# Vi-Sri/CerebralSignalNetworks

Hardware: AMD Instinct MI355X
Metric: EEG-segments/sec training (128ch x 500, hidden=768) (higher is better)
Workload: dtype bf16

## Files before the change

### cerebralsignalnetworks_amd/csrc/csn_common.h

```cpp
#pragma once
#include <hip/hip_runtime.h>
#include <stdint.h>
#include <stdio.h>
#include <stdlib.h>
#include <atomic>
#include <string>

#include "../../include/csn_hip.h"

namespace csn {

typedef __bf16 bf16_t;
typedef __attribute__((ext_vector_type(8))) __bf16 bf16x8;
typedef __attribute__((ext_vector_type(4))) __bf16 bf16x4;
typedef __attribute__((ext_vector_type(4))) float f32x4;
typedef __attribute__((ext_vector_type(4))) short s16x4;

void set_error(const std::string& msg);
int fail(int status, const char* fmt, ...);

#define CSN_HIP_CHECK(expr)                                                              \
  do {                                                                                   \
    hipError_t _e = (expr);                                                              \
    if (_e != hipSuccess)                                                                \
      return ::csn::fail(CSN_ERR_HIP, "%s failed: %s (%s:%d)", #expr, hipGetErrorString(_e), \
                         __FILE__, __LINE__);                                            \
  } while (0)

#define CSN_LAUNCH_CHECK()                                                               \
  do {                                                                                   \
    hipError_t _e = hipGetLastError();                                                   \
    if (_e != hipSuccess)                                                                \
      return ::csn::fail(CSN_ERR_HIP, "kernel launch failed: %s (%s:%d)",                \
                         hipGetErrorString(_e), __FILE__, __LINE__);                     \
  } while (0)

#define CSN_REQUIRE(cond, ...)                                                           \
  do {                                                                                   \
    if (!(cond)) return ::csn::fail(CSN_ERR_INVALID_ARGUMENT, __VA_ARGS__);              \
  } while (0)

struct Options {
  bool cell_v1, no_persist, no_persist_bwd, persist_streams, no_xcd_local, no_rotate, no_fuse_x, no_beside,
      no_side_stream, fwd_ksplit, fwd_nsplit, fwd_flags, bwd_flags, dpoll_no_hint, fwd_hint, gemm_no_dma, gemm_no_256, gemm_generic, tn_no_tr, tn_no_stagger, filter_v1, tags_no_rearm, gemm_no_192, no_half_tiles, nt_no_w4, no_fwd_park;
  int chunk;
  int tn_stages;
};
static inline Options options_from_env() {
  auto on = [](const char* name) { return getenv(name) != nullptr; };
  auto num = [](const char* name, int dflt) {
    const char* e = getenv(name);
    return e ? atoi(e) : dflt;
  };
  Options o{};
  o.cell_v1 = on("CSN_CELL_V1");
  o.no_persist = on("CSN_NO_PERSIST");
  o.no_persist_bwd = on("CSN_NO_PERSIST_BWD");
  o.persist_streams = on("CSN_PERSIST_STREAMS");
  o.no_xcd_local = on("CSN_NO_XCD_LOCAL");
  o.no_rotate = on("CSN_NO_ROTATE");
  o.no_fuse_x = on("CSN_NO_FUSE_X");
  o.no_beside = on("CSN_NO_BESIDE");
  o.no_half_tiles = on("CSN_NO_HALF_TILES");
  o.no_fwd_park = on("CSN_NO_FWD_PARK");
  o.no_side_stream = on("CSN_NO_SIDE_STREAM");
  o.fwd_ksplit = on("CSN_FWD_KSPLIT");
  o.fwd_nsplit = on("CSN_FWD_NSPLIT");
  o.fwd_flags = on("CSN_FWD_FLAGS");
  o.bwd_flags = on("CSN_BWD_FLAGS");
  o.dpoll_no_hint = on("CSN_DPOLL_NO_HINT");
  o.fwd_hint = on("CSN_FWD_HINT");
  o.tn_no_stagger = on("CSN_TN_NO_STAGGER");
  o.gemm_no_dma = on("CSN_GEMM_NO_DMA");
  o.gemm_no_256 = on("CSN_GEMM_NO_256");
  o.gemm_no_192 = on("CSN_GEMM_NO_192");
  o.nt_no_w4 = on("CSN_NT_NO_W4");
  o.gemm_generic = on("CSN_GEMM_GENERIC");
  o.tn_no_tr = on("CSN_TN_NO_TR");
  o.filter_v1 = on("CSN_FILTER_V1");
#ifdef CSN_SLAB_TAGS
  o.tags_no_rearm = on("CSN_TAGS_NO_REARM");
#endif
  o.chunk = num("CSN_LSTM_CHUNK", 32);
  if (o.chunk < 1) o.chunk = 1;
  o.tn_stages = num("CSN_TN_STAGES", 4);
  return o;
}
// ... 73 lines not shown
```

### cerebralsignalnetworks_amd/csrc/lstm.hip

```cpp
#include <algorithm>
#include <cstring>
#include <vector>

#include "csn_common.h"
#include "lstm_cell_blk.h"
#include "lstm_cell_common.h"
#include "lstm_dropout.h"
#include "lstm_f32_persist.h"
#include "lstm_resident.h"

namespace csn {

struct LayerWs {
  size_t wih, whh, whht, wiht, whh_blk, whht_blk, bias, xproj, gates, c_all, h_all, dgates, dx, dc_carry, hblk[2],
      dgblk[2], h_blk_all, counters, dg_blk_all, bflags;
  size_t h_drop;
};
struct WsLayout {
  LayerWs layer[8];
  size_t x_c, x_blk, wih0_blk, dy_tm, tn_scratch, colsum, status, agree, agree_b, zeros_bh, f32_bias_part, total;
  size_t zero_fwd, zero_fwd_bytes, zero_bwd, zero_bwd_bytes;
  bool fuse_x;
  bool il, persist, persist_bwd;
  bool fwd_ns;
  bool f32_persist;
};

static bool whole_chip() {
  int dev = 0, cus = 0;
  if (hipGetDevice(&dev) != hipSuccess) return false;
  return hipDeviceGetAttribute(&cus, hipDeviceAttributeMultiprocessorCount, dev) == hipSuccess && cus >= 256;
}

static WsLayout make_layout(const csnLstmDesc& d, int training, bool dropout, const Options& opt) {
  WsLayout w{};
  w.il = cell_blk_supported(d.H, d.dtype, opt);
  const bool slabs_fit = ((size_t)d.T + 1) * (((size_t)d.B + 63) / 64 * 64) * (size_t)d.H * 8 < ((size_t)1 << 32);
  w.fwd_ns = w.il && fwd_ns_supported(d.B, d.H, d.dtype, opt) && d.L <= 4;
  w.persist = w.fwd_ns || (w.il && slabs_fit && fwd_persist_supported(d.B, d.H, d.dtype, opt) && d.L <= 4);
  w.persist_bwd = w.persist && slabs_fit && training && bwd_persist_supported(d.B, d.H, d.dtype, opt);
  size_t off = 0;
  const size_t es = dtype_size(d.dtype);
  auto take = [&](size_t bytes) {
    size_t o = off;
    off += align_up(bytes, 256);
    return o;
  };
  const size_t TB = (size_t)d.T * d.B, H = d.H, G = 4 * (size_t)d.H;
  const size_t Bpad = ((size_t)d.B + 63) / 64 * 64;
  size_t tn_bytes = 0;
  for (int l = 0; l < d.L; ++l) {
    const size_t I = l == 0 ? d.I : d.H;
    LayerWs& L = w.layer[l];
    L.wih = take(G * I * es);
    L.wiht = take(G * I * es);
    L.bias = take(G * 4);
    if (w.il) {
      L.whh_blk = take(G * H * 2);
      L.whht_blk = take(G * H * 2);
      L.hblk[0] = take(Bpad * H * 2);
      L.hblk[1] = take(Bpad * H * 2);
      if (w.persist) L.h_blk_all = take(((size_t)(d.T < 3 ? 3 : d.T) + 1) * Bpad * H * 2);
    } else {
      L.whh = take(G * H * es);
      L.whht = take(G * H * es);
    }
    L.xproj = take(TB * G * 4);
    L.gates = take(TB * G * es);
    L.c_all = take((TB + d.B) * H * 4);
    L.h_all = take((TB + d.B) * H * es);
    if (training) {
      L.dgates = take(TB * G * es);
      L.dx = take(TB * I * 4);
      if (!w.persist_bwd) L.dc_carry = take((size_t)d.B * H * 4);
      if (w.il) {
        L.dgblk[0] = take(Bpad * G * 2);
        L.dgblk[1] = take(Bpad * G * 2);
      }
      if (w.persist_bwd) L.dg_blk_all = take((size_t)(d.T < 4 ? 4 : d.T) * Bpad * G * 2);
    }
    size_t a = gemm_tn_scratch_bytes(G, I, TB, opt), b = gemm_tn_scratch_bytes(G, H, TB, opt);
    if (a > tn_bytes) tn_bytes = a;
    if (b > tn_bytes) tn_bytes = b;
  }
  w.x_c = take(TB * d.I * es);
  w.status = take(256);
  w.fuse_x = w.persist && !opt.no_fuse_x &&
             (w.fwd_ns ? d.I == 128 : (d.I % 32 == 0 && d.I <= 128 && d.H != 512));
  if (w.fuse_x) {
    w.x_blk = take((size_t)d.T * Bpad * d.I * 2);
    w.wih0_blk = take(G * d.I * 2);
  }
  if (w.persist_bwd) w.zeros_bh = take((size_t)d.B * H * 4);
  w.f32_persist = !w.il && d.dtype == CSN_F32 && !opt.no_persist && !opt.cell_v1 && f32_persist_supported(d.B, d.H) && whole_chip();
  if (w.f32_persist) {
    const size_t MTt = Bpad / 64;
    w.zero_fwd = off;
    for (int l = 0; l < d.L; ++l) w.layer[l].counters = take(((size_t)d.T + 1) * MTt * kF32FlagLine * 4);
    w.zero_fwd_bytes = off - w.zero_fwd;
    for (int l = 0; l < d.L; ++l) w.layer[l].h_blk_all = take(((size_t)d.T + 1) * Bpad * H * 4);
    if (training) {
      for (int l = 0; l < d.L; ++l) w.layer[l].dg_blk_all = take((size_t)d.T * Bpad * G * 4);
      w.zeros_bh = take((size_t)d.B * H * 4);
      w.f32_bias_part = take(MTt * 4 * G * 4);
      w.zero_bwd = off;
// ... 2 lines not shown
    }
  }
  if (w.persist) {
    w.zero_fwd = off;
    for (int l = 0; l < d.L; ++l) w.layer[l].counters = take(((size_t)d.T + 1) * (Bpad / 64) * 4 * kPersistFlagLine * 4);
    w.agree = take(((size_t)d.T + 8) * 8 * sizeof(unsigned long long));
    w.zero_fwd_bytes = off - w.zero_fwd;
  }
  if (w.persist_bwd) {
    w.zero_bwd = off;
    for (int l = 0; l < d.L; ++l) {
      w.layer[l].dc_carry = take((size_t)d.B * H * 4);
      w.layer[l].bflags = take((size_t)d.T * (Bpad / 64) * 3 * kPersistFlagLine * 4);
    }
    w.agree_b = take(((size_t)d.T + 8) * 8 * sizeof(unsigned long long));
    w.zero_bwd_bytes = off - w.zero_bwd;
  }
  if (training) {
    w.dy_tm = take(TB * H * 4);
    w.tn_scratch = take(tn_bytes);
    w.colsum = take(colsum_scratch_bytes(G));
  }
  for (int l = 0; dropout && l + 1 < d.L; ++l) w.layer[l].h_drop = take(TB * H * es);
  w.total = off;
  return w;
}

static const int kPlanBits = CSN_LSTM_STATE | CSN_LSTM_DROPOUT | CSN_LSTM_REVERSE | CSN_LSTM_RESIDENT;

static int check_resident(const char* fn, const csnLstmDesc* d, int training) {
  if ((training & CSN_LSTM_RESIDENT) && !resident_supported(d->H))
    return fail(CSN_ERR_UNSUPPORTED, "%s: CSN_LSTM_RESIDENT takes H <= %d, not H=%d", fn, kResidentMaxH, d->H);
  return CSN_OK;
}
static void resident_options(Options& opt) {
  opt.cell_v1 = true;
  opt.no_persist = true;
}

static int check_desc(const char* fn, const csnLstmDesc* d) {
  CSN_REQUIRE(d != nullptr, "%s: null descriptor", fn);
  CSN_REQUIRE(d->B > 0 && d->T > 0 && d->I > 0 && d->H > 0, "%s: bad shape B=%d T=%d I=%d H=%d", fn, d->B, d->T,
              d->I, d->H);
  CSN_REQUIRE(d->L >= 1 && d->L <= 8, "%s: L=%d outside 1..8", fn, d->L);
  CSN_REQUIRE(d->H % 32 == 0, "%s: H=%d must be a multiple of 32", fn, d->H);
  CSN_REQUIRE(d->dtype == CSN_F32 || d->dtype == CSN_BF16, "%s: bad dtype %d", fn, d->dtype);
// ... 681 lines not shown
  return CSN_OK;
}

static bool drop_on(const Call& C) { return C.P.dropout && C.P.drop_p > 0.f && C.NL > 1; }
static const void* layer_input(const Call& C, int l) {
  if (l > 0 && drop_on(C)) return C.ws + C.w.layer[l - 1].h_drop;
  return l == 0 ? (const void*)(C.ws + C.w.x_c) : (const void*)(C.ws + C.w.layer[l - 1].h_all + (size_t)C.B * C.H * C.es);
}

static int drop_fwd(const Call& C, int l, int t_lo, int t_hi, hipStream_t on) {
  if (!drop_on(C)) return CSN_OK;
  const size_t BH = (size_t)C.B * C.H;
  return launch_lstm_dropout_fwd(C.ws + C.w.layer[l].h_all + (size_t)(t_lo + 1) * BH * C.es, C.ws + C.w.layer[l].h_drop + (size_t)t_lo * BH * C.es,
                                 (int64_t)(t_hi - t_lo + 1) * (int64_t)BH, ((uint64_t)l * C.T_full + t_lo) * BH, C.dt,
                                 dropout_cfg(C.P.drop_p, C.P.drop_seed, C.P.drop_subsequence), on);
}
static int drop_bwd(const Call& C, int l, int t_lo, int t_hi, hipStream_t on) {
  if (!drop_on(C)) return CSN_OK;
  const size_t BH = (size_t)C.B * C.H;
  return launch_lstm_dropout_bwd((float*)(C.ws + C.w.layer[l + 1].dx) + (size_t)t_lo * BH, (int64_t)(t_hi - t_lo + 1) * (int64_t)BH,
                                 ((uint64_t)l * C.T_full + t_lo) * BH, dropout_cfg(C.P.drop_p, C.P.drop_seed, C.P.drop_subsequence), on);
}

static int install_slot0(const Call& C, int l, const float* h0, const float* c0) {
  const LayerWs& L = C.w.layer[l];
  const size_t BH = (size_t)C.B * C.H;
  if (h0) {
    if (int rc = launch_cast(h0 + l * BH, C.ws + L.h_all, (int64_t)BH, C.dt, C.st)) return rc;
  } else {
    CSN_HIP_CHECK(hipMemsetAsync(C.ws + L.h_all, 0, BH * C.es, C.st));
  }
  if (c0)
    CSN_HIP_CHECK(hipMemcpyAsync(C.ws + L.c_all, c0 + l * BH, BH * 4, hipMemcpyDeviceToDevice, C.st));
  else
    CSN_HIP_CHECK(hipMemsetAsync(C.ws + L.c_all, 0, BH * 4, C.st));
  return CSN_OK;
}

static int seed_dc_carry(const Call& C, int l, const float* dc_n, bool zeroed) {
  const size_t BH = (size_t)C.B * C.H;
  if (dc_n)
    CSN_HIP_CHECK(hipMemcpyAsync(C.ws + C.w.layer[l].dc_carry, dc_n + l * BH, BH * 4, hipMemcpyDeviceToDevice, C.st));
  else if (!zeroed)
    CSN_HIP_CHECK(hipMemsetAsync(C.ws + C.w.layer[l].dc_carry, 0, BH * 4, C.st));
  return CSN_OK;
}

static int prep_row_major(const Call& C, const FwdArgs& A) {
  const WsLayout& w = C.w;
  char* ws = C.ws;
  hipStream_t st = C.st;
  const int H = C.H, dt = C.dt;
  const int64_t G = C.G;
  int rc;
  if ((rc = launch_cast_strided(A.x, A.xsb, A.xst, C.B, C.T, C.d.I, ws + w.x_c, dt, st, C.dlen, C.P.reverse, C.vrow, C.vt0))) return rc;
  if ((rc = mask_x(C, st))) return rc;
  for (int l = 0; l < C.NL; ++l) {
// ... 46 lines not shown

static int weight_grads_rm(const Call& C, const BwdArgs& A, int l, bool colsum) {
  const WsLayout& w = C.w;
  const LayerWs& L = w.layer[l];
  char* ws = C.ws;
  const int acc = C.P.grad_accumulate;
  int rc;
  if ((rc = gemm_tn_full(ws + L.dgates, ws + L.h_all, A.dw_hh[l], C.G, C.H, C.TB, C.dt, ws + w.tn_scratch, acc, C.st, C.P.opt))) return rc;
  if ((rc = gemm_tn_full(ws + L.dgates, layer_input(C, l), A.dw_ih[l], C.G, C.in_width(l), C.TB, C.dt, ws + w.tn_scratch, acc, C.st, C.P.opt))) return rc;
  if (colsum) return launch_colsum(ws + L.dgates, C.TB, C.G, C.dt, A.db_ih[l], A.db_hh[l], acc, ws + w.colsum, C.st);
  return CSN_OK;
}

static int weight_grads_blk(const Call& C, const BwdArgs& A, int l, hipStream_t on) {
  const WsLayout& w = C.w;
  const LayerWs& L = w.layer[l];
  char* ws = C.ws;
  const int H = C.H;
  const int64_t G = C.G, TB = C.TB, I = C.in_width(l);
  float* slabs = (float*)(ws + w.tn_scratch);
  const int acc = C.P.grad_accumulate;
  int S = 1, r;
  int cs_done = 0, S_cs = 1;
  if ((r = launch_gemm_tn_slabs(ws + L.dgates, ws + L.h_all, slabs, G, H, TB, CSN_BF16, on, &S, (float*)(ws + w.colsum), &cs_done, C.P.opt))) return r;
  S_cs = S;
  if ((r = launch_reduce_slabs_unperm(slabs, G * H, S, H, H, A.dw_hh[l], nullptr, acc, on))) return r;
  if ((r = launch_gemm_tn_slabs(ws + L.dgates, layer_input(C, l), slabs, G, I, TB, CSN_BF16, on, &S, nullptr, nullptr, C.P.opt))) return r;
  if ((r = launch_reduce_slabs_unperm(slabs, G * I, S, H, I, A.dw_ih[l], nullptr, acc, on))) return r;
  if (!cs_done) {
    if ((r = launch_colsum_partial(ws + L.dgates, TB, G, CSN_BF16, ws + w.colsum, on))) return r;
    S_cs = colsum_chunks();
  }
  return launch_reduce_slabs_unperm((const float*)(ws + w.colsum), G, S_cs, H, 1, A.db_ih[l], A.db_hh[l], acc, on);
}

static int prof_end(Call& C, int k, int launches, int cells) {
  Prof& g_prof = C.P.prof;
  if (int rc = prof_mark(g_prof, 2 * k + 1, C.st)) return rc;
  g_prof.launches[k] = launches;
  g_prof.cells[k] = cells;
  g_prof.have[k] = g_prof.on;
  return CSN_OK;
}

static int launch_dh0(const Call& C, int l, float* out) {
  const LayerWs& L = C.w.layer[l];
// ... 262 lines not shown
    a.B = B; a.T = T; a.MT_total = MTt;
    for (int m = 0; m < MTt; m += per) {
      a.mt0 = m;
      a.MT = MTt - m < per ? MTt - m : per;
      if ((rc = prof_pair(g_prof, 1, false, st))) return rc;
      if ((rc = launch_bwd_f32_persist(a, H, st))) return rc;
      if ((rc = prof_pair(g_prof, 1, true, st))) return rc;
      ++n_launch;
    }
    sum_rows_kernel<<<(unsigned)((G + 255) / 256), 256, 0, st>>>((const float*)(ws + w.f32_bias_part), MTt * 4, G, A.db_ih[l], A.db_hh[l], C.P.grad_accumulate);
    CSN_LAUNCH_CHECK();
    if (l > 0 && (rc = gemm_nt(ws + L.dgates, ws + L.wiht, nullptr, ws + L.dx, C.TB, H, G, CSN_F32, CSN_F32, 0, st, C.P.opt))) return rc;
    if (l > 0 && (rc = drop_bwd(C, l - 1, 0, T - 1, st))) return rc;
  }
  if ((rc = prof_end(C, 1, n_launch, T * NL))) return rc;
  for (int l = NL - 1; l >= 0; --l) {
    if ((rc = weight_grads_rm(C, A, l, false))) return rc;
    C.P.grads_ready(l);
  }
  if (A.dx) return dx_out(C, A.dx, st);
  return CSN_OK;
}

static int prep_fast(Call& C, const FwdArgs& A) {
  const csnLstmDesc& d = C.d;
  const WsLayout& w = C.w;
  char* ws = C.ws;
  hipStream_t st = C.st;
  const int B = C.B, T = C.T, H = C.H, NL = C.NL;
  const int64_t G = C.G, TB = C.TB;
  const size_t Bpad = ((size_t)B + 63) / 64 * 64;
  int rc;
  PrepArgs pa{};
  pa.vrow = C.vrow;
  pa.vt0 = C.vt0;
  int prep_rc = CSN_OK;
  auto job = [&](int kind, const float* a_, const float* b_, void* dst, int64_t n0, int64_t n1, int64_t n2, int64_t s0,
                 int64_t s1, int64_t Hh, int pr, int pk, int64_t work) {
    if (prep_rc != CSN_OK) return;
    if (pa.njobs == kPrepMaxJobs) {
      if ((prep_rc = launch_prep_multi(pa, st)) != CSN_OK) return;
      pa.njobs = 0;
    }
    PrepJob& J = pa.job[pa.njobs++];
    J = PrepJob{kind, a_, b_, dst, n0, n1, n2, s0, s1, Hh, pr, pk, work, 0u, 0u, nullptr};
  };
  job(kPrepCastX, A.x, nullptr, ws + w.x_c, B, T, d.I, A.xsb, A.xst, 0, C.P.reverse, 0, TB * d.I);
  pa.job[pa.njobs - 1].len = C.dlen;
  for (int l = 0; l < NL; ++l) {
    const LayerWs& L = w.layer[l];
    const int64_t I = C.in_width(l);
    job(kPrepPermRows, A.w_ih[l], nullptr, ws + L.wih, 0, I, 0, 0, 0, H, 0, 0, G * I);
    job(kPrepBlockify, A.w_hh[l], nullptr, ws + L.whh_blk, G, H, 0, H, 1, H, 1, 0, G * H / 8);
    job(kPrepBias, A.b_ih[l], A.b_hh[l], ws + L.bias, 0, 0, 0, 0, 0, H, 0, 0, G);
    if (C.P.training) {
      job(kPrepTransPerm, A.w_ih[l], nullptr, ws + L.wiht, 0, I, 0, 0, 0, H, 0, 0, G * I);
      job(kPrepBlockify, A.w_hh[l], nullptr, ws + L.whht_blk, H, G, 0, 1, H, H, 0, 1, H * G / 8);
    }
    if (!w.persist) {
      CSN_HIP_CHECK(hipMemsetAsync(ws + L.hblk[0], 0, Bpad * H * 2, st));
      CSN_HIP_CHECK(hipMemsetAsync(ws + L.hblk[1], 0, Bpad * H * 2, st));
      if (A.h0 && (rc = launch_blockify_x(A.h0 + (size_t)l * B * H, H, 0, B, 1, H, ws + L.hblk[0], st))) return rc;
      if ((rc = install_slot0(C, l, A.h0, A.c0))) return rc;
    }
  }
  if (w.fuse_x) {
    job(kPrepBlockifyX, A.x, nullptr, ws + w.x_blk, B, T, d.I, A.xsb, A.xst, (int64_t)Bpad, C.P.reverse, 0, (int64_t)T * Bpad * d.I / 8);
    pa.job[pa.njobs - 1].len = C.dlen;
    job(kPrepBlockify, A.w_ih[0], nullptr, ws + w.wih0_blk, G, d.I, 0, d.I, 1, H, 1, 0, G * d.I / 8);
  }
  if (prep_rc != CSN_OK) return prep_rc;
  if ((rc = launch_prep_multi(pa, st))) return rc;
  if ((rc = mask_x(C, st))) return rc;
  if (!w.fuse_x) {
    if ((rc = gemm_nt(ws + w.x_c, ws + w.layer[0].wih, (const float*)(ws + w.layer[0].bias), ws + w.layer[0].xproj,
                      TB, G, d.I, CSN_BF16, CSN_F32, 0, st, C.P.opt)))
      return rc;
  }
  return CSN_OK;
}

static int forward_il(Call& C, const FwdArgs& A) {
  const WsLayout& w = C.w;
  char* ws = C.ws;
  hipStream_t st = C.st;
  SideCtx* sc = &C.P.sc;
  int rc;
  if ((rc = side_ctx(C.P.sc))) return rc;
  hipStream_t side = C.P.opt.no_side_stream ? st : sc->side;
  const int B = C.B, T = C.T, H = C.H, NL = C.NL;
  const int64_t G = C.G;
  const int Cz = C.Cz, lag = 2 * Cz;
  const int training = C.P.training;
// ... 47 lines not shown
      xproj_ready[(size_t)(l + 1) * nch + c] = ev;
    }
  }
  return prof_end(C, 0, n_launch, n_cells);
}

static int forward_persist(Call& C, const FwdArgs& A) {
  Plan& P = C.P;
  const WsLayout& w = C.w;
  Prof& g_prof = P.prof;
  char* ws = C.ws;
  hipStream_t st = C.st;
  SideCtx* sc = &P.sc;
  int rc;
  if ((rc = side_ctx(P.sc))) return rc;
  hipStream_t side = P.opt.no_side_stream ? st : sc->side;
  const float* h0 = A.h0;
  const float* c0 = A.c0;
  const int B = C.B, T = C.T, H = C.H, NL = C.NL;
  const int Bpad = (B + 63) / 64 * 64, MT = Bpad / 64;
  const int Cz = C.Cz;
  const int nch = (T + Cz - 1) / Cz;
  const int training = P.training;
  if ((rc = prep_fast(C, A))) return rc;
  CSN_HIP_CHECK(hipMemsetAsync(ws + w.zero_fwd, 0, w.zero_fwd_bytes, st));
  auto fill_slot = [&](PersistFwdSlot& S, int l, int c) {
    const LayerWs& L = w.layer[l];
    S.w_blk = (const bf16_t*)(ws + L.whh_blk);
    S.xproj = (const float*)(ws + L.xproj);
    S.gates = training ? (bf16_t*)(ws + L.gates) : nullptr;
    S.c_all = (float*)(ws + L.c_all);
    S.h_all = (bf16_t*)(ws + L.h_all);
    S.h_blk_all = (bf16_t*)(ws + L.h_blk_all);
    S.flags = (unsigned*)(ws + L.counters);
    S.x_blk = nullptr;
    S.wih_blk = nullptr;
    S.bias = nullptr;
    S.I = 0;
    if (l == 0 && w.fuse_x) {
      S.x_blk = (const bf16_t*)(ws + w.x_blk);
      S.wih_blk = (const bf16_t*)(ws + w.wih0_blk);
      S.bias = (const float*)(ws + L.bias);
      S.I = C.d.I;
    }
    const Chunk k = chunk_at(C, c);
    S.t0 = k.t0;
    S.nsteps = k.nsteps;
  };
  PersistFwdArgs a{};
  a.error_flag = (unsigned*)(ws + w.status);
  a.B = B; a.H = H; a.T = T; a.Bpad = Bpad; a.MT = MT;
  a.rotate = !P.opt.no_rotate;
  a.park = !P.opt.no_fwd_park;
  a.data_polls = (!w.fwd_ns && !P.opt.fwd_flags) ? (P.opt.fwd_hint && !P.opt.dpoll_no_hint ? 1 : 2) : 0;
#ifdef CSN_SLAB_TAGS
  if (a.data_polls && P.opt.tags_no_rearm) a.data_polls |= 4;
#endif
  if (a.data_polls)
    for (int l = 0; l < NL; ++l)
      CSN_HIP_CHECK(hipMemsetAsync(ws + w.layer[l].h_blk_all, 0xff, (size_t)4 * Bpad * H * 2, st));
  a.state = (h0 || c0) ? 1 : 0;
  if (a.state) P.state_seen = true;
  for (int l = 0; l < NL && P.state_seen; ++l) {
    const LayerWs& L = w.layer[l];
    if (h0) {
      if ((rc = launch_blockify_x(h0 + (size_t)l * B * H, H, 0, B, 1, H, ws + L.h_blk_all, st))) return rc;
    } else if (a.state) {
      CSN_HIP_CHECK(hipMemsetAsync(ws + L.h_blk_all, 0, (size_t)Bpad * H * 2, st));
    }
    if ((rc = install_slot0(C, l, h0, c0))) return rc;
  }
  int n_launch = 0;
  P.half_launches[0] = 0;

  const int max_slots = NL < nch ? NL : nch;
  const int fwd_slices = w.fwd_ns ? fwd_ns_slices(H) : fwd_persist_slices(H);
  auto launch_fwd = [&](const PersistFwdArgs& args, hipStream_t on) {
    return w.fwd_ns ? launch_fwd_ns(args, on) : launch_fwd_persist(args, on);
  };
  const bool grouped = max_slots <= 4 && max_slots * MT <= 8 && fwd_slices <= 32 &&
                       !P.opt.persist_streams;
  if (grouped) {
    const int ndiag = nch + NL - 1;
    const bool try_local = !P.opt.no_xcd_local;
    if ((rc = prof_mark(g_prof, 0, st))) return rc;
    for (int dg = 0; dg < ndiag; ++dg) {
      int lay[4], chk[4], ns = 0;
      for (int l = 0; l < NL; ++l) {
        const int c = dg - l;
        if (c < 0 || c >= nch) continue;
        lay[ns] = l;
        chk[ns] = c;
        fill_slot(a.slot[ns], l, c);
// ... 141 lines not shown
  }
  if ((rc = prof_end(C, 1, n_launch, n_cells))) return rc;
  if ((rc = hand_off(sc, side, st))) return rc;
  for (int l = NL - 1; l >= 0; --l) C.P.grads_ready(l);
  return CSN_OK;
}

static int backward_persist(Call& C, const BwdArgs& A) {
  Plan& P = C.P;
  const WsLayout& w = C.w;
  Prof& g_prof = P.prof;
  char* ws = C.ws;
  hipStream_t st = C.st;
  const float* dh_n = A.dh_n;
  const int B = C.B, T = C.T, H = C.H, NL = C.NL;
  const int64_t G = C.G;
  const int Bpad = (B + 63) / 64 * 64, MT = Bpad / 64;
  const int Cz = C.Cz;
  const int nch = (T + Cz - 1) / Cz;
  const bool beside = NL > 1 && NL <= 4 && bwd_persist_slices(H) <= 28 && G % 64 == 0 && !P.opt.no_beside;
  const int lag = beside ? 2 : 1;
  const int ndiag = nch + lag * (NL - 1);
  int rc;
  CSN_HIP_CHECK(hipMemsetAsync(ws + w.zero_bwd, 0, w.zero_bwd_bytes, st));
  for (int l = 0; l < NL; ++l)
    if ((rc = seed_dc_carry(C, l, A.dc_n, true))) return rc;
  struct DhAdd { int l, t_lo, t_hi; };
  auto add_dh_n = [&](const DhAdd& q) -> int {
    return add_dh_n_rows(C, dh_n + (size_t)(q.l - 1) * B * H, (float*)(ws + w.layer[q.l].dx), q.t_lo, q.t_hi, st);
  };
  const bool try_local = !P.opt.no_xcd_local;

  PersistBwdArgs a{};
  a.error_flag = (unsigned*)(ws + w.status);
  a.B = B; a.H = H; a.T = T; a.Bpad = Bpad; a.MT = MT;
  a.xcd_groups = 1;
  a.grid_slices = 32;
  a.rotate = !P.opt.no_rotate;
  a.data_polls = P.opt.bwd_flags ? 0 : (P.opt.dpoll_no_hint ? 2 : 1);
#ifdef CSN_SLAB_TAGS
  if (a.data_polls && P.opt.tags_no_rearm) a.data_polls |= 4;
#endif
  P.dgates_copies = 2;
  if (a.data_polls)
    for (int l = 0; l < NL; ++l) CSN_HIP_CHECK(hipMemsetAsync(ws + w.layer[l].dg_blk_all, 0xff, (size_t)4 * Bpad * G * 2, st));
  int n_launch = 0;
  P.half_launches[1] = 0;
  BesideGemm pending[3];
  DhAdd pending_add[3] = {{0, 0, 0}, {0, 0, 0}, {0, 0, 0}};
  DhAdd pending_drop[3] = {{0, 0, 0}, {0, 0, 0}, {0, 0, 0}};
  int npending = 0;
  if ((rc = prof_mark(g_prof, 2, st))) return rc;
  for (int dg = 0; dg < ndiag; ++dg) {
    int lay[4], chk[4], ns = 0;
    for (int l = NL - 1; l >= 0; --l) {
      const int c = dg - lag * (NL - 1 - l);
      if (c < 0 || c >= nch) continue;
      const LayerWs& L = w.layer[l];
      PersistBwdSlot& S = a.slot[ns];
      S.wt_blk = (const bf16_t*)(ws + L.whht_blk);
      S.gates = (const bf16_t*)(ws + L.gates);
      S.c_all = (const float*)(ws + L.c_all);
      if (l == NL - 1) {
        S.dy = A.dy_tm;
        S.dy_last = A.dy_tm ? nullptr : A.dy_last;
      } else {
        S.dy = (const float*)(ws + w.layer[l + 1].dx);
// ... 330 lines not shown
```

### cerebralsignalnetworks_amd/csrc/lstm_cell_blk.h

```cpp
#pragma once
#include "csn_common.h"

#ifdef CSN_SLAB_TAGS
#define CSN_DPOLL_MODE(x) ((x) & 3)
#define CSN_DPOLL_NO_REARM(x) (((x) & 4) != 0)
#else
#define CSN_DPOLL_MODE(x) (x)
#define CSN_DPOLL_NO_REARM(x) false
#endif

namespace csn {

struct CellFwdProb {
  const bf16_t* h_prev_blk;
  const bf16_t* w_blk;
  const float* xproj;
  const float* c_prev;
  bf16_t* gates_out;
  float* c_out;
  bf16_t* h_out;
  bf16_t* h_out_blk;
};
struct CellFwdArgs {
  CellFwdProb p[4];
// ... 74 lines not shown
  bf16_t* dgates;
  bf16_t* dg_blk_all;
  unsigned* flags;
  int t_hi, nsteps;
};
struct PersistBwdArgs {
  PersistBwdSlot slot[4];
  int nslots;
  BesideGemm gemm[3];
  int ngemm;
  int grid_slices;
  int xcd_groups;
  int rotate;
  int data_polls;
  unsigned long long* agree;
  unsigned* error_flag;
  int B, H, T, Bpad, MT;
  int half_tiles;
};
bool bwd_persist_supported(int B, int H, int dtype, const Options& opt);
int bwd_persist_slices(int H);
int launch_bwd_persist(const PersistBwdArgs& a, hipStream_t st, const int* lengths = nullptr);

enum { kPrepBlockify = 0, kPrepPermRows, kPrepTransPerm, kPrepBias, kPrepCastX, kPrepBlockifyX };
static constexpr int kPrepMaxJobs = 32;
struct PrepJob {
  int kind;
  const float* a;
  const float* b;
  void* dst;
  int64_t n0, n1, n2, s0, s1, H;
  int perm_r, perm_k;
  int64_t work;
  unsigned blk_begin, blk_count;
  const int* len;
};
struct PrepArgs {
  PrepJob job[kPrepMaxJobs];
  int njobs;
  const int* vrow;
  const int* vt0;
};
static_assert(sizeof(PrepArgs) <= 4096, "PrepArgs is passed by value: the kernel-argument segment holds 4096 bytes");
int launch_prep_multi(PrepArgs& A, hipStream_t st);

bool cell_blk_supported(int H, int dtype, const Options& opt);
int launch_cell_fwd_il(const CellFwdArgs& a, int nprob, hipStream_t st);
int launch_cell_bwd_il(const CellBwdArgs& a, int nprob, hipStream_t st, const CellMask* mask = nullptr);
int launch_blockify_x(const float* x, int64_t xsb, int64_t xst, int B, int T, int I, void* dst, hipStream_t st);
int launch_blockify(const float* src, int64_t ld_r, int64_t ld_k, int64_t R, int64_t K, int perm_r, int perm_k,
                    int64_t H, void* dst, hipStream_t st);
int launch_permute_rows_cast(const float* src, int64_t H, int64_t I, void* dst, hipStream_t st);
int launch_transpose_perm_cast(const float* src, int64_t H, int64_t I, void* dst, hipStream_t st);
int launch_bias_perm_sum(const float* a, const float* b, int64_t H, float* dst, hipStream_t st);
int launch_reduce_slabs_unperm(const float* slabs, int64_t slab_stride, int S, int64_t H, int64_t C, float* out,
                               float* out2, int accumulate, hipStream_t st);

}
```

### cerebralsignalnetworks_amd/csrc/lstm_cell_blk.hip

```cpp
#include "csn_common.h"
#include "lstm_cell_common.h"
#include "lstm_cell_blk.h"

#ifdef CSN_STAMPS
__device__ unsigned long long* g_stamps = nullptr;
#define CSN_STAMP(i)                                                                      \
  do {                                                                                    \
    __builtin_amdgcn_sched_barrier(0);                                                    \
    if (threadIdx.x == 0)                                                                 \
      g_stamps[((blockIdx.z * gridDim.y + blockIdx.y) * gridDim.x + blockIdx.x) * 8 + (i)] = wall_clock64(); \
    __builtin_amdgcn_sched_barrier(0);                                                    \
  } while (0)
#else
#define CSN_STAMP(i)
#endif

namespace csn {

__device__ __forceinline__ int64_t std_row(int64_t nprime, int64_t H) { return (nprime & 3) * H + (nprime >> 2); }

__global__ void __launch_bounds__(256)
blockify_cast_kernel(const float* __restrict__ src, int64_t ld_r, int64_t ld_k, int64_t R, int64_t K, int perm_r,
                     int perm_k, int64_t H, bf16_t* __restrict__ dst) {
  const int64_t nchunks = R * K / 8;
// ... 30 lines not shown
    const int64_t c = i / G, n = i % G;
    dst[i] = (bf16_t)src[std_row(n, H) * I + c];
  }
}

__global__ void bias_perm_sum_kernel(const float* __restrict__ a, const float* __restrict__ b, int64_t H,
                                     float* __restrict__ dst) {
  const int64_t i = (int64_t)blockIdx.x * blockDim.x + threadIdx.x;
  if (i < 4 * H) dst[i] = a[std_row(i, H)] + b[std_row(i, H)];
}

__global__ void reduce_slabs_unperm_kernel(const float* __restrict__ slabs, int64_t slab_stride, int S, int64_t H,
                                           int64_t C, float* out, float* out2, int accumulate) {
  const int64_t total = 4 * H * C;
  const int64_t stride = (int64_t)gridDim.x * blockDim.x;
  for (int64_t i = (int64_t)blockIdx.x * blockDim.x + threadIdx.x; i < total; i += stride) {
    const int64_t n = i / C, c = i % C;
    float acc = 0.0f;
    for (int s = 0; s < S; ++s) acc += slabs[(int64_t)s * slab_stride + i];
    const int64_t o = std_row(n, H) * C + c;
    out[o] = accumulate ? out[o] + acc : acc;
    if (out2 != nullptr) out2[o] = accumulate ? out2[o] + acc : acc;
  }
}

__global__ void __launch_bounds__(256) prep_multi_kernel(PrepArgs A) {
  __shared__ __attribute__((aligned(16))) bf16_t tp[64][72];
  int j = 0;
  while (j + 1 < A.njobs && blockIdx.x >= A.job[j + 1].blk_begin) ++j;
  const PrepJob& J = A.job[j];
  const int64_t vb = blockIdx.x - J.blk_begin, vg = J.blk_count;
  const int64_t gid = vb * blockDim.x + threadIdx.x, stride = vg * blockDim.x;
  switch (J.kind) {
    case kPrepBlockify: {
      const int64_t R = J.n0, K = J.n1, H = J.H, ld_r = J.s0, ld_k = J.s1, kblocks = K >> 5;
      bf16_t* dst = (bf16_t*)J.dst;
      if (J.perm_k && !J.perm_r && ld_r == 1 && (R & 63) == 0 && (K & 63) == 0 && (ld_k & 3) == 0) {
        const int64_t tiles_u = R >> 6, ntiles = tiles_u * (K >> 6);
        const int t = threadIdx.x, rr = t >> 2, seg = t & 3;
        for (int64_t tile = vb; tile < ntiles; tile += vg) {
          const int64_t tu = tile % tiles_u, tk = tile / tiles_u;
          const float4* sp = reinterpret_cast<const float4*>(J.a + std_row(tk * 64 + rr, H) * ld_k + tu * 64 + seg * 16);
          const float4 q0 = sp[0], q1 = sp[1], q2 = sp[2], q3 = sp[3];
          *reinterpret_cast<bf16x8*>(&tp[rr][seg * 16]) = (bf16x8){(bf16_t)q0.x, (bf16_t)q0.y, (bf16_t)q0.z, (bf16_t)q0.w, (bf16_t)q1.x, (bf16_t)q1.y, (bf16_t)q1.z, (bf16_t)q1.w};
          *reinterpret_cast<bf16x8*>(&tp[rr][seg * 16 + 8]) = (bf16x8){(bf16_t)q2.x, (bf16_t)q2.y, (bf16_t)q2.z, (bf16_t)q2.w, (bf16_t)q3.x, (bf16_t)q3.y, (bf16_t)q3.z, (bf16_t)q3.w};
          __syncthreads();
// ... 130 lines not shown
          if (J.perm_r) t = n - 1 - t;
          if (t < 0 || (win && t >= n)) {
            *reinterpret_cast<uint4*>(dst + ci * 8) = make_uint4(0u, 0u, 0u, 0u);
            continue;
          }
          if (win) {
            sr = A.vrow[r];
            t += A.vt0[r];
          }
        }
        bf16x8 v;
        if (r < Bn && ((J.s0 | J.s1) & 3) == 0 && (reinterpret_cast<uintptr_t>(J.a) & 15) == 0) {
          const float4* sp = reinterpret_cast<const float4*>(J.a + sr * J.s0 + t * J.s1 + k);
          const float4 u = sp[0], w = sp[1];
          v = (bf16x8){(bf16_t)u.x, (bf16_t)u.y, (bf16_t)u.z, (bf16_t)u.w, (bf16_t)w.x, (bf16_t)w.y, (bf16_t)w.z, (bf16_t)w.w};
        } else {
#pragma unroll
          for (int e = 0; e < 8; ++e) v[e] = (bf16_t)(r < Bn ? J.a[sr * J.s0 + t * J.s1 + k + e] : 0.f);
        }
        *reinterpret_cast<bf16x8*>(dst + ci * 8) = v;
      }
      break;
    }
  }
}

int launch_prep_multi(PrepArgs& A, hipStream_t st) {
  CSN_REQUIRE(A.njobs >= 1 && A.njobs <= kPrepMaxJobs, "launch_prep_multi: %d jobs", A.njobs);
  unsigned total = 0;
  for (int j = 0; j < A.njobs; ++j) {
    int64_t blocks = (A.job[j].work + 255) / 256;
    if (blocks < 1) blocks = 1;
    if (blocks > 2048) blocks = 2048;
    A.job[j].blk_begin = total;
    A.job[j].blk_count = (unsigned)blocks;
    total += (unsigned)blocks;
  }
  prep_multi_kernel<<<total, 256, 0, st>>>(A);
  CSN_LAUNCH_CHECK();
  return CSN_OK;
}

static inline unsigned cap_grid(int64_t n) {
  int64_t g = (n + 255) / 256;
  return (unsigned)(g < 1 ? 1 : (g > 2048 ? 2048 : g));
}

// ... 381 lines not shown
```

Before: 27960.

## Fuse workspace memsets into prep kernel and batch weight-gradient slab reductions

Folds the forward workspace zero/0xff memsets into the existing multi-job prep kernel, and merges the backward memsets into a single multi-region fill kernel. In the backward weight-gradient path, both TN GEMMs now write to separate slab buffers so that the dW_hh, dW_ih and bias reductions run in one launch with a vectorized slab-sum kernel. This aims to cut the launch count and serialization per step, at the cost of an extra scratch buffer and more complex job dispatch.

New measurement: 27900 (median of 2 runs). About the same (-0.2%).

```diff
diff --git a/cerebralsignalnetworks_amd/csrc/csn_common.h b/cerebralsignalnetworks_amd/csrc/csn_common.h
--- a/cerebralsignalnetworks_amd/csrc/csn_common.h
+++ b/cerebralsignalnetworks_amd/csrc/csn_common.h
@@ -42,7 +42,7 @@
 
 struct Options {
   bool cell_v1, no_persist, no_persist_bwd, persist_streams, no_xcd_local, no_rotate, no_fuse_x, no_beside,
-      no_side_stream, fwd_ksplit, fwd_nsplit, fwd_flags, bwd_flags, dpoll_no_hint, fwd_hint, gemm_no_dma, gemm_no_256, gemm_generic, tn_no_tr, tn_no_stagger, filter_v1, tags_no_rearm, gemm_no_192, no_half_tiles, nt_no_w4, no_fwd_park;
+      no_side_stream, fwd_ksplit, fwd_nsplit, fwd_flags, bwd_flags, dpoll_no_hint, fwd_hint, gemm_no_dma, gemm_no_256, gemm_generic, tn_no_tr, tn_no_stagger, filter_v1, tags_no_rearm, gemm_no_192, no_half_tiles, nt_no_w4, no_fwd_park, no_fill_fuse, no_reduce_fuse;
   int chunk;
   int tn_stages;
 };
@@ -63,6 +63,8 @@
   o.no_beside = on("CSN_NO_BESIDE");
   o.no_half_tiles = on("CSN_NO_HALF_TILES");
   o.no_fwd_park = on("CSN_NO_FWD_PARK");
+  o.no_fill_fuse = on("CSN_NO_FILL_FUSE");
+  o.no_reduce_fuse = on("CSN_NO_REDUCE_FUSE");
   o.no_side_stream = on("CSN_NO_SIDE_STREAM");
   o.fwd_ksplit = on("CSN_FWD_KSPLIT");
   o.fwd_nsplit = on("CSN_FWD_NSPLIT");
diff --git a/cerebralsignalnetworks_amd/csrc/lstm.hip b/cerebralsignalnetworks_amd/csrc/lstm.hip
--- a/cerebralsignalnetworks_amd/csrc/lstm.hip
+++ b/cerebralsignalnetworks_amd/csrc/lstm.hip
@@ -19,6 +19,7 @@
 struct WsLayout {
   LayerWs layer[8];
   size_t x_c, x_blk, wih0_blk, dy_tm, tn_scratch, colsum, status, agree, agree_b, zeros_bh, f32_bias_part, total;
+  size_t tn_scratch2;
   size_t zero_fwd, zero_fwd_bytes, zero_bwd, zero_bwd_bytes;
   bool fuse_x;
   bool il, persist, persist_bwd;
@@ -48,7 +49,7 @@
   };
   const size_t TB = (size_t)d.T * d.B, H = d.H, G = 4 * (size_t)d.H;
   const size_t Bpad = ((size_t)d.B + 63) / 64 * 64;
-  size_t tn_bytes = 0;
+  size_t tn_bytes = 0, tn2_bytes = 0;
   for (int l = 0; l < d.L; ++l) {
     const size_t I = l == 0 ? d.I : d.H;
     LayerWs& L = w.layer[l];
@@ -81,6 +82,7 @@
     }
     size_t a = gemm_tn_scratch_bytes(G, I, TB, opt), b = gemm_tn_scratch_bytes(G, H, TB, opt);
     if (a > tn_bytes) tn_bytes = a;
+    if (a > tn2_bytes) tn2_bytes = a;
     if (b > tn_bytes) tn_bytes = b;
   }
   w.x_c = take(TB * d.I * es);
@@ -129,6 +131,7 @@
     w.colsum = take(colsum_scratch_bytes(G));
   }
   for (int l = 0; dropout && l + 1 < d.L; ++l) w.layer[l].h_drop = take(TB * H * es);
+  if (w.persist_bwd && !opt.no_reduce_fuse) w.tn_scratch2 = take(tn2_bytes);
   w.total = off;
   return w;
 }
@@ -856,17 +859,17 @@
                                  ((uint64_t)l * C.T_full + t_lo) * BH, dropout_cfg(C.P.drop_p, C.P.drop_seed, C.P.drop_subsequence), on);
 }
 
-static int install_slot0(const Call& C, int l, const float* h0, const float* c0) {
+static int install_slot0(const Call& C, int l, const float* h0, const float* c0, bool zeroed = false) {
   const LayerWs& L = C.w.layer[l];
   const size_t BH = (size_t)C.B * C.H;
   if (h0) {
     if (int rc = launch_cast(h0 + l * BH, C.ws + L.h_all, (int64_t)BH, C.dt, C.st)) return rc;
-  } else {
+  } else if (!zeroed) {
     CSN_HIP_CHECK(hipMemsetAsync(C.ws + L.h_all, 0, BH * C.es, C.st));
   }
   if (c0)
     CSN_HIP_CHECK(hipMemcpyAsync(C.ws + L.c_all, c0 + l * BH, BH * 4, hipMemcpyDeviceToDevice, C.st));
-  else
+  else if (!zeroed)
     CSN_HIP_CHECK(hipMemsetAsync(C.ws + L.c_all, 0, BH * 4, C.st));
   return CSN_OK;
 }
@@ -959,6 +962,24 @@
   const int acc = C.P.grad_accumulate;
   int S = 1, r;
   int cs_done = 0, S_cs = 1;
+  if (w.tn_scratch2 != 0) {
+    float* slabs2 = (float*)(ws + w.tn_scratch2);
+    int S2 = 1;
+    if ((r = launch_gemm_tn_slabs(ws + L.dgates, ws + L.h_all, slabs, G, H, TB, CSN_BF16, on, &S, (float*)(ws + w.colsum), &cs_done, C.P.opt))) return r;
+    S_cs = S;
+    if ((r = launch_gemm_tn_slabs(ws + L.dgates, layer_input(C, l), slabs2, G, I, TB, CSN_BF16, on, &S2, nullptr, nullptr, C.P.opt))) return r;
+    if (!cs_done) {
+      if ((r = launch_colsum_partial(ws + L.dgates, TB, G, CSN_BF16, ws + w.colsum, on))) return r;
+      S_cs = colsum_chunks();
+    }
+    ReduceArgs ra{};
+    ra.njobs = 3;
+    ra.accumulate = acc;
+    ra.job[0] = ReduceJob{slabs, G * H, A.dw_hh[l], nullptr, H, H, S, 0, 0u, 0u, 0u};
+    ra.job[1] = ReduceJob{slabs2, G * I, A.dw_ih[l], nullptr, H, I, S2, 0, 0u, 0u, 0u};
+    ra.job[2] = ReduceJob{(const float*)(ws + w.colsum), G, A.db_ih[l], A.db_hh[l], H, 1, S_cs, 0, 0u, 0u, 0u};
+    return launch_reduce_multi_unperm(ra, on);
+  }
   if ((r = launch_gemm_tn_slabs(ws + L.dgates, ws + L.h_all, slabs, G, H, TB, CSN_BF16, on, &S, (float*)(ws + w.colsum), &cs_done, C.P.opt))) return r;
   S_cs = S;
   if ((r = launch_reduce_slabs_unperm(slabs, G * H, S, H, H, A.dw_hh[l], nullptr, acc, on))) return r;
@@ -1267,7 +1288,7 @@
   return CSN_OK;
 }
 
-static int prep_fast(Call& C, const FwdArgs& A) {
+static int prep_fast(Call& C, const FwdArgs& A, const FillJob* fills = nullptr, int nfills = 0) {
   const csnLstmDesc& d = C.d;
   const WsLayout& w = C.w;
   char* ws = C.ws;
@@ -1314,6 +1335,8 @@
     pa.job[pa.njobs - 1].len = C.dlen;
     job(kPrepBlockify, A.w_ih[0], nullptr, ws + w.wih0_blk, G, d.I, 0, d.I, 1, H, 1, 0, G * d.I / 8);
   }
+  for (int i = 0; i < nfills; ++i)
+    job(kPrepFill, nullptr, nullptr, fills[i].dst, fills[i].bytes, fills[i].value, 0, 0, 0, 0, 0, 0, fills[i].bytes / 16 + 1);
   if (prep_rc != CSN_OK) return prep_rc;
   if ((rc = launch_prep_multi(pa, st))) return rc;
   if ((rc = mask_x(C, st))) return rc;
@@ -1407,8 +1430,30 @@
   const int Cz = C.Cz;
   const int nch = (T + Cz - 1) / Cz;
   const int training = P.training;
-  if ((rc = prep_fast(C, A))) return rc;
-  CSN_HIP_CHECK(hipMemsetAsync(ws + w.zero_fwd, 0, w.zero_fwd_bytes, st));
+  int data_polls = (!w.fwd_ns && !P.opt.fwd_flags) ? (P.opt.fwd_hint && !P.opt.dpoll_no_hint ? 1 : 2) : 0;
+#ifdef CSN_SLAB_TAGS
+  if (data_polls && P.opt.tags_no_rearm) data_polls |= 4;
+#endif
+  const bool state = h0 || c0;
+  if (state) P.state_seen = true;
+  const bool fuse_fills = !P.opt.no_fill_fuse;
+  const size_t slab = (size_t)Bpad * H * 2, BH = (size_t)B * H;
+  FillJob fills[kFillMaxJobs];
+  int nfills = 0;
+  auto fill = [&](size_t off, size_t bytes, int value) { fills[nfills++] = FillJob{ws + off, (int64_t)bytes, value, 0u, 0u}; };
+  if (fuse_fills) {
+    fill(w.zero_fwd, w.zero_fwd_bytes, 0);
+    for (int l = 0; l < NL; ++l) {
+      const LayerWs& L = w.layer[l];
+      const bool zero0 = state && !h0;
+      if (zero0) fill(L.h_blk_all, slab, 0);
+      if (data_polls) fill(L.h_blk_all + (zero0 ? slab : 0), (zero0 ? 3 : 4) * slab, 0xff);
+      if (P.state_seen && !h0) fill(L.h_all, BH * C.es, 0);
+      if (P.state_seen && !c0) fill(L.c_all, BH * 4, 0);
+    }
+  }
+  if ((rc = prep_fast(C, A, fills, nfills))) return rc;
+  if (!fuse_fills) CSN_HIP_CHECK(hipMemsetAsync(ws + w.zero_fwd, 0, w.zero_fwd_bytes, st));
   auto fill_slot = [&](PersistFwdSlot& S, int l, int c) {
     const LayerWs& L = w.layer[l];
     S.w_blk = (const bf16_t*)(ws + L.whh_blk);
@@ -1437,23 +1482,19 @@
   a.B = B; a.H = H; a.T = T; a.Bpad = Bpad; a.MT = MT;
   a.rotate = !P.opt.no_rotate;
   a.park = !P.opt.no_fwd_park;
-  a.data_polls = (!w.fwd_ns && !P.opt.fwd_flags) ? (P.opt.fwd_hint && !P.opt.dpoll_no_hint ? 1 : 2) : 0;
-#ifdef CSN_SLAB_TAGS
-  if (a.data_polls && P.opt.tags_no_rearm) a.data_polls |= 4;
-#endif
-  if (a.data_polls)
+  a.data_polls = data_polls;
+  if (a.data_polls && !fuse_fills)
     for (int l = 0; l < NL; ++l)
-      CSN_HIP_CHECK(hipMemsetAsync(ws + w.layer[l].h_blk_all, 0xff, (size_t)4 * Bpad * H * 2, st));
-  a.state = (h0 || c0) ? 1 : 0;
-  if (a.state) P.state_seen = true;
+      CSN_HIP_CHECK(hipMemsetAsync(ws + w.layer[l].h_blk_all, 0xff, 4 * slab, st));
+  a.state = state ? 1 : 0;
   for (int l = 0; l < NL && P.state_seen; ++l) {
     const LayerWs& L = w.layer[l];
     if (h0) {
       if ((rc = launch_blockify_x(h0 + (size_t)l * B * H, H, 0, B, 1, H, ws + L.h_blk_all, st))) return rc;
-    } else if (a.state) {
-      CSN_HIP_CHECK(hipMemsetAsync(ws + L.h_blk_all, 0, (size_t)Bpad * H * 2, st));
-    }
-    if ((rc = install_slot0(C, l, h0, c0))) return rc;
+    } else if (a.state && !fuse_fills) {
+      CSN_HIP_CHECK(hipMemsetAsync(ws + L.h_blk_all, 0, slab, st));
+    }
+    if ((rc = install_slot0(C, l, h0, c0, fuse_fills))) return rc;
   }
   int n_launch = 0;
   P.half_launches[0] = 0;
@@ -1641,7 +1682,16 @@
   const int lag = beside ? 2 : 1;
   const int ndiag = nch + lag * (NL - 1);
   int rc;
-  CSN_HIP_CHECK(hipMemsetAsync(ws + w.zero_bwd, 0, w.zero_bwd_bytes, st));
+  const bool fuse_fills = !P.opt.no_fill_fuse;
+  if (fuse_fills) {
+    FillArgs fa{};
+    fa.job[fa.njobs++] = FillJob{ws + w.zero_bwd, (int64_t)w.zero_bwd_bytes, 0, 0u, 0u};
+    for (int l = 0; l < NL && !P.opt.bwd_flags; ++l)
+      fa.job[fa.njobs++] = FillJob{ws + w.layer[l].dg_blk_all, (int64_t)4 * Bpad * G * 2, 0xff, 0u, 0u};
+    if ((rc = launch_fill_multi(fa, st))) return rc;
+  } else {
+    CSN_HIP_CHECK(hipMemsetAsync(ws + w.zero_bwd, 0, w.zero_bwd_bytes, st));
+  }
   for (int l = 0; l < NL; ++l)
     if ((rc = seed_dc_carry(C, l, A.dc_n, true))) return rc;
   struct DhAdd { int l, t_lo, t_hi; };
@@ -1661,7 +1711,7 @@
   if (a.data_polls && P.opt.tags_no_rearm) a.data_polls |= 4;
 #endif
   P.dgates_copies = 2;
-  if (a.data_polls)
+  if (a.data_polls && !fuse_fills)
     for (int l = 0; l < NL; ++l) CSN_HIP_CHECK(hipMemsetAsync(ws + w.layer[l].dg_blk_all, 0xff, (size_t)4 * Bpad * G * 2, st));
   int n_launch = 0;
   P.half_launches[1] = 0;
diff --git a/cerebralsignalnetworks_amd/csrc/lstm_cell_blk.h b/cerebralsignalnetworks_amd/csrc/lstm_cell_blk.h
--- a/cerebralsignalnetworks_amd/csrc/lstm_cell_blk.h
+++ b/cerebralsignalnetworks_amd/csrc/lstm_cell_blk.h
@@ -120,7 +120,7 @@
 int bwd_persist_slices(int H);
 int launch_bwd_persist(const PersistBwdArgs& a, hipStream_t st, const int* lengths = nullptr);
 
-enum { kPrepBlockify = 0, kPrepPermRows, kPrepTransPerm, kPrepBias, kPrepCastX, kPrepBlockifyX };
+enum { kPrepBlockify = 0, kPrepPermRows, kPrepTransPerm, kPrepBias, kPrepCastX, kPrepBlockifyX, kPrepFill };
 static constexpr int kPrepMaxJobs = 32;
 struct PrepJob {
   int kind;
@@ -142,6 +142,36 @@
 static_assert(sizeof(PrepArgs) <= 4096, "PrepArgs is passed by value: the kernel-argument segment holds 4096 bytes");
 int launch_prep_multi(PrepArgs& A, hipStream_t st);
 
+static constexpr int kFillMaxJobs = 16;
+struct FillJob {
+  void* dst;
+  int64_t bytes;
+  int value;
+  unsigned blk_begin, blk_count;
+};
+struct FillArgs {
+  FillJob job[kFillMaxJobs];
+  int njobs;
+};
+int launch_fill_multi(FillArgs& A, hipStream_t st);
+
+struct ReduceJob {
+  const float* slabs;
+  int64_t slab_stride;
+  float* out;
+  float* out2;
+  int64_t H, C;
+  int S;
+  int vec;
+  unsigned rows_per_blk, blk_begin, blk_count;
+};
+struct ReduceArgs {
+  ReduceJob job[3];
+  int njobs;
+  int accumulate;
+};
+int launch_reduce_multi_unperm(ReduceArgs& A, hipStream_t st);
+
 bool cell_blk_supported(int H, int dtype, const Options& opt);
 int launch_cell_fwd_il(const CellFwdArgs& a, int nprob, hipStream_t st);
 int launch_cell_bwd_il(const CellBwdArgs& a, int nprob, hipStream_t st, const CellMask* mask = nullptr);
diff --git a/cerebralsignalnetworks_amd/csrc/lstm_cell_blk.hip b/cerebralsignalnetworks_amd/csrc/lstm_cell_blk.hip
--- a/cerebralsignalnetworks_amd/csrc/lstm_cell_blk.hip
+++ b/cerebralsignalnetworks_amd/csrc/lstm_cell_blk.hip
@@ -76,6 +76,77 @@
     out[o] = accumulate ? out[o] + acc : acc;
     if (out2 != nullptr) out2[o] = accumulate ? out2[o] + acc : acc;
   }
+}
+
+template <int N, typename T>
+__device__ __forceinline__ void add_slabs(T& acc, const T* p, int64_t sv) {
+  T v[N];
+#pragma unroll
+  for (int j = 0; j < N; ++j) v[j] = p[j * sv];
+#pragma unroll
+  for (int j = 0; j < N; ++j) acc += v[j];
+}
+template <typename T>
+__device__ __forceinline__ void reduce_job(const ReduceJob& J, int accumulate, unsigned vb) {
+  constexpr int V = sizeof(T) / 4;
+  const unsigned cols = (unsigned)J.C / V;
+  const unsigned rl = threadIdx.x / cols, c0 = threadIdx.x - rl * cols;
+  if (rl >= J.rows_per_blk) return;
+  const unsigned rows = 4u * (unsigned)J.H, S = (unsigned)J.S;
+  const int64_t sv = J.slab_stride / V;
+  for (unsigned n = vb * J.rows_per_blk + rl; n < rows; n += J.blk_count * J.rows_per_blk) {
+    const int64_t o_row = std_row(n, J.H) * J.C;
+    for (unsigned c = c0; c < cols; c += 256) {
+      const T* p = reinterpret_cast<const T*>(J.slabs + (int64_t)n * J.C) + c;
+      T acc{};
+      unsigned s = 0;
+      for (; s + 8 <= S; s += 8) add_slabs<8>(acc, p + s * sv, sv);
+      switch (S - s) {
+        case 7: add_slabs<7>(acc, p + s * sv, sv); break;
+        case 6: add_slabs<6>(acc, p + s * sv, sv); break;
+        case 5: add_slabs<5>(acc, p + s * sv, sv); break;
+        case 4: add_slabs<4>(acc, p + s * sv, sv); break;
+        case 3: add_slabs<3>(acc, p + s * sv, sv); break;
+        case 2: add_slabs<2>(acc, p + s * sv, sv); break;
+        case 1: add_slabs<1>(acc, p + s * sv, sv); break;
+        default: break;
+      }
+      T* o = reinterpret_cast<T*>(J.out + o_row) + c;
+      *o = accumulate ? *o + acc : acc;
+      if (J.out2 != nullptr) {
+        T* o2 = reinterpret_cast<T*>(J.out2 + o_row) + c;
+        *o2 = accumulate ? *o2 + acc : acc;
+      }
+    }
+  }
+}
+__global__ void __launch_bounds__(256) reduce_multi_unperm_kernel(ReduceArgs A) {
+  int j = 0;
+  while (j + 1 < A.njobs && blockIdx.x >= A.job[j + 1].blk_begin) ++j;
+  const ReduceJob& J = A.job[j];
+  const unsigned vb = blockIdx.x - J.blk_begin;
+  if (J.vec)
+    reduce_job<f32x4>(J, A.accumulate, vb);
+  else
+    reduce_job<float>(J, A.accumulate, vb);
+}
+
+__device__ __forceinline__ void fill_region(char* dst, int64_t bytes, int value, int64_t gid, int64_t stride) {
+  const unsigned b = (unsigned)value & 0xffu, w = b * 0x01010101u;
+  int64_t head = (int64_t)((16 - (reinterpret_cast<uintptr_t>(dst) & 15)) & 15);
+  if (head > bytes) head = bytes;
+  const int64_t nvec = (bytes - head) >> 4, tail = bytes - head - (nvec << 4);
+  uint4* body = reinterpret_cast<uint4*>(dst + head);
+  for (int64_t i = gid; i < nvec; i += stride) body[i] = make_uint4(w, w, w, w);
+  if (gid < head) dst[gid] = (char)b;
+  if (gid < tail) dst[head + (nvec << 4) + gid] = (char)b;
+}
+__global__ void __launch_bounds__(256) fill_multi_kernel(FillArgs A) {
+  int j = 0;
+  while (j + 1 < A.njobs && blockIdx.x >= A.job[j + 1].blk_begin) ++j;
+  const FillJob& J = A.job[j];
+  fill_region((char*)J.dst, J.bytes, J.value, (int64_t)(blockIdx.x - J.blk_begin) * blockDim.x + threadIdx.x,
+              (int64_t)J.blk_count * blockDim.x);
 }
 
 __global__ void __launch_bounds__(256) prep_multi_kernel(PrepArgs A) {
@@ -252,7 +323,47 @@
       }
       break;
     }
-  }
+    case kPrepFill:
+      fill_region((char*)J.dst, J.n0, (int)J.n1, gid, stride);
+      break;
+  }
+}
+
+int launch_fill_multi(FillArgs& A, hipStream_t st) {
+  CSN_REQUIRE(A.njobs >= 1 && A.njobs <= kFillMaxJobs, "launch_fill_multi: %d jobs", A.njobs);
+  unsigned total = 0;
+  for (int j = 0; j < A.njobs; ++j) {
+    int64_t blocks = (A.job[j].bytes / 16 + 255) / 256;
+    if (blocks < 1) blocks = 1;
+    if (blocks > 2048) blocks = 2048;
+    A.job[j].blk_begin = total;
+    A.job[j].blk_count = (unsigned)blocks;
+    total += (unsigned)blocks;
+  }
+  fill_multi_kernel<<<total, 256, 0, st>>>(A);
+  CSN_LAUNCH_CHECK();
+  return CSN_OK;
+}
+
+int launch_reduce_multi_unperm(ReduceArgs& A, hipStream_t st) {
+  CSN_REQUIRE(A.njobs >= 1 && A.njobs <= 3, "launch_reduce_multi_unperm: %d jobs", A.njobs);
+  unsigned total = 0;
+  for (int j = 0; j < A.njobs; ++j) {
+    ReduceJob& J = A.job[j];
+    CSN_REQUIRE(J.S >= 1 && J.H >= 1 && J.C >= 1 && J.C <= (1 << 28), "launch_reduce_multi_unperm: job %d", j);
+    const uintptr_t bits = reinterpret_cast<uintptr_t>(J.slabs) | reinterpret_cast<uintptr_t>(J.out) | reinterpret_cast<uintptr_t>(J.out2);
+    J.vec = (J.C & 3) == 0 && (bits & 15) == 0;
+    const int64_t cols = J.C / (J.vec ? 4 : 1);
+    J.rows_per_blk = cols >= 256 ? 1u : (unsigned)(256 / cols);
+    int64_t blocks = (4 * J.H + J.rows_per_blk - 1) / J.rows_per_blk;
+    if (blocks > 4096) blocks = 4096;
+    J.blk_begin = total;
+    J.blk_count = (unsigned)blocks;
+    total += (unsigned)blocks;
+  }
+  reduce_multi_unperm_kernel<<<total, 256, 0, st>>>(A);
+  CSN_LAUNCH_CHECK();
+  return CSN_OK;
 }
 
 int launch_prep_multi(PrepArgs& A, hipStream_t st) {
```
